# ardaduz/deep-video-mvs

Hardware: AMD Instinct MI355X
Metric: depth frames/sec/GPU @ 320x256x64 planes (fusionnet); rel-L1 vs ref (higher is better)
Workload: dtype f32

## Files before the change

deep-video-mvs_amd/csrc/direct_conv.hip:

```cpp
#include <stdlib.h>

#include "dvmvs_device.h"

namespace dvmvs {

typedef float float4v __attribute__((ext_vector_type(4)));

struct DirectConvArgs {
  const float* x;
  const float* packed;
  const float* bias;
  float* dst;
  float* dst_nhwc;
  long long x_batch_stride, dst_batch_stride;
  int B, C_in, C_out, H, W, OH, OW;
  int act;
  int n_groups;
  int packed_groups;
  int n_chunks;
  int tiles_x;
  int vec4;
};

#ifdef DVMVS_SWEEP_TRACE
// ... 320 lines not shown
}

template <int PX>
__global__ __launch_bounds__(256) void conv_head_kernel(const float* __restrict__ x, const float* __restrict__ w, const float* __restrict__ bias,
                                                        float* __restrict__ dst, long long x_batch_stride, long long dst_batch_stride, int C, int H,
                                                        int W, int act, float p0, float p1) {
  constexpr int SL = 256 / PX;
  __shared__ float s_part[SL][PX];
  const int px = threadIdx.x % PX, slice = threadIdx.x / PX;
  const int HW = H * W;
  const int p = blockIdx.x * PX + px, b = blockIdx.y;
  const int y = p / W, xx = p - y * W;
  const int per = (C + SL - 1) / SL;
  const int c_lo = slice * per, c_hi = min(C, c_lo + per);
  float sum = 0.0f;
  if (p < HW) {
    int off[9];
    bool in[9];
#pragma unroll
    for (int t = 0; t < 9; ++t) {
      const int yy = y + t / 3 - 1, xs = xx + t % 3 - 1;
      in[t] = yy >= 0 && yy < H && xs >= 0 && xs < W;
      off[t] = in[t] ? yy * W + xs : 0;
    }
    const float* xb = x + static_cast<size_t>(b) * x_batch_stride;
#pragma unroll 2
    for (int c = c_lo; c < c_hi; ++c) {
      const float* plane = xb + static_cast<size_t>(c) * HW;
      float v[9];
#pragma unroll
      for (int t = 0; t < 9; ++t) v[t] = in[t] ? plane[off[t]] : 0.0f;
#pragma unroll
      for (int t = 0; t < 9; ++t) sum = fmaf(v[t], w[c * 9 + t], sum);
    }
  }
  s_part[slice][px] = sum;
  __syncthreads();
  if (slice == 0 && p < HW) {
    float total = s_part[0][px];
#pragma unroll
    for (int s = 1; s < SL; ++s) total += s_part[s][px];
    if (bias) total += bias[0];
    dst[static_cast<size_t>(b) * dst_batch_stride + p] = head_activation(total, act, p0, p1);
  }
}

struct DirectConvShape {
  int MW, MT, NT, PW, KS;
};
constexpr DirectConvShape kDcShapes[4] = {{16, 5, 2, 4, 2}, {8, 5, 2, 1, 8}, {16, 5, 1, 1, 8}, {8, 5, 1, 1, 8}};
constexpr int kDcCUs = 256;

inline int direct_conv_choose(int B, int C_in, int C_out, int H, int W, int K, int S) {
  if (B <= 0 || C_in <= 0 || C_out <= 0 || C_out % 16 != 0 || (K != 3 && K != 5) || (S != 1 && S != 2) || H <= 0 || W <= 0) return 0;
  if (S == 2 && (H % 2 != 0 || W % 2 != 0)) return 0;
  const int OH = H / S, OW = W / S;
// ... 110 lines not shown
  a.n_chunks = 0; a.tiles_x = 0;
  hipStream_t s = static_cast<hipStream_t>(stream);
  if (kernel_size == 3) return stride == 1 ? launch_direct_conv_shape<3, 1>(id, a, s) : launch_direct_conv_shape<3, 2>(id, a, s);
  return stride == 1 ? launch_direct_conv_shape<5, 1>(id, a, s) : launch_direct_conv_shape<5, 2>(id, a, s);
}

extern "C" int dvmvs_conv_head_fwd(const float* x, long long x_batch_stride, const float* weight, const float* bias, float* dst,
                                   long long dst_batch_stride, int B, int C_in, int H, int W, int activation, float p0, float p1, dvmvs_stream_t stream) {
  using namespace dvmvs;
  if (!x || !weight || !dst || B <= 0 || C_in <= 0 || H <= 0 || W <= 0) return DVMVS_EINVAL;
  if (activation < 0 || activation > 3) return DVMVS_EINVAL;
  const long long HW = static_cast<long long>(H) * W;
  if (x_batch_stride == 0) x_batch_stride = HW * C_in;
  if (dst_batch_stride == 0) dst_batch_stride = HW;
  hipStream_t s = static_cast<hipStream_t>(stream);
  if (HW >= 16384) {
    hipLaunchKernelGGL((conv_head_kernel<64>), dim3(static_cast<unsigned int>((HW + 63) / 64), B), dim3(256), 0, s, x, weight, bias, dst, x_batch_stride,
                       dst_batch_stride, C_in, H, W, activation, p0, p1);
  } else {
    hipLaunchKernelGGL((conv_head_kernel<16>), dim3(static_cast<unsigned int>((HW + 15) / 16), B), dim3(256), 0, s, x, weight, bias, dst, x_batch_stride,
                       dst_batch_stride, C_in, H, W, activation, p0, p1);
  }
  return launch_status();
}

#ifdef DVMVS_SWEEP_TRACE
extern "C" int dvmvs_debug_direct_conv_trace(unsigned long long* host, int waves) {
  if (waves > dvmvs::kDcTraceWaves) waves = dvmvs::kDcTraceWaves;
  return static_cast<int>(hipMemcpyFromSymbol(host, HIP_SYMBOL(dvmvs::g_dc_trace), sizeof(unsigned long long) * dvmvs::kDcTraceWords * waves));
}
#endif
// ... 1 lines not shown
```

deep-video-mvs_amd/csrc/dvmvs_device.h:

```cpp
#pragma once

#include <hip/hip_runtime.h>
#include <stdint.h>

#include "../../include/dvmvs_hip.h"

namespace dvmvs {

constexpr int kWave = 64;

#define DVMVS_GLOBAL __attribute__((address_space(1)))
typedef const float DVMVS_GLOBAL* gcfloat_p;
typedef float DVMVS_GLOBAL* gfloat_p;
typedef unsigned int DVMVS_GLOBAL* guint_p;
__device__ inline gcfloat_p as_global(const float* p) { return (gcfloat_p)p; }
__device__ inline gfloat_p as_global(float* p) { return (gfloat_p)p; }
__device__ inline guint_p as_global(unsigned int* p) { return (guint_p)p; }

#define DVMVS_RETURN_IF_HIP(expr)                      \
  do {                                                 \
    hipError_t _e = (expr);                            \
    if (_e != hipSuccess) return static_cast<int>(_e); \
  } while (0)

// ... 90 lines not shown
  const float ey = (fy + 1.0f) - ay;
  const float wy = ay - fy;
  t.w_nw = ex * ey;
  t.w_ne = wx * ey;
  t.w_sw = ex * wy;
  t.w_se = wx * wy;
  t.in_x0 = (t.x0 >= 0) && (t.x0 < W);
  t.in_x1 = (t.x0 + 1 >= 0) && (t.x0 + 1 < W);
  t.in_y0 = (t.y0 >= 0) && (t.y0 < H);
  t.in_y1 = (t.y0 + 1 >= 0) && (t.y0 + 1 < H);
  return t;
}

__device__ inline float unnormalize_ac(float g, int size) { return ((g + 1.0f) * 0.5f) * static_cast<float>(size - 1); }

__device__ inline int wave_inclusive_scan(int x) {
  const int lane = threadIdx.x & 63;
#pragma unroll
  for (int off = 1; off < 64; off <<= 1) {
    const int y = __shfl_up(x, off, 64);
    if (lane >= off) x += y;
  }
  return x;
}

template <int kBlock = 256>
__device__ inline int block_exclusive_scan(int v, int* lds, int& total) {
  const int incl = wave_inclusive_scan(v);
  const int wave = threadIdx.x >> 6;
  if ((threadIdx.x & 63) == 63) lds[wave] = incl;
// ... 41 lines not shown
```

deep-video-mvs_amd/csrc/frame_ops.hip:

```cpp
#include "dvmvs_device.h"

namespace dvmvs {

template <int ACT>
__device__ inline float apply_act(float v, float p0 = 0.0f, float p1 = 0.0f) {
  if (ACT == 1) return fmaxf(v, 0.0f);
  if (ACT == 2) return 1.0f / (1.0f + expf(-v));
  if (ACT == 3) {
#pragma clang fp contract(off)
    const float s = 1.0f / (1.0f + expf(-v));
    return 1.0f / (p0 * s + p1);
  }
  return v;
}

template <int ACT, bool VEC4, int RES>
__global__ __launch_bounds__(256) void bias_act_kernel(const float* x, float* dst, long long dst_batch_stride, const float* __restrict__ bias,
                                                       const float* __restrict__ residual, int C, int HW, int W, float p0, float p1) {
  const int plane = blockIdx.y;
  const int b = plane / C, c = plane - b * C;
  const float bv = bias ? bias[c] : 0.0f;
  const float* p = x + static_cast<size_t>(plane) * HW;
  float* d = dst + static_cast<size_t>(b) * dst_batch_stride + static_cast<size_t>(c) * HW;
  if (VEC4 && RES != 2) {
// ... 44 lines not shown
    const long long pl = i / (static_cast<long long>(OW) * OH);
    const float fy = sh * static_cast<float>(oy), fx = sw * static_cast<float>(ox);
    const int y0 = static_cast<int>(fy), x0 = static_cast<int>(fx);
    const int y1 = y0 + (y0 < H - 1 ? 1 : 0), x1 = x0 + (x0 < W - 1 ? 1 : 0);
    const float h1 = fy - static_cast<float>(y0), h0 = 1.0f - h1;
    const float w1 = fx - static_cast<float>(x0), w0 = 1.0f - w1;
    const float* p = in + pl * H * W;
    const long long b = pl / C, c = pl - b * C;
    const float bv = (PRE != 0 && pre_bias) ? pre_bias[c] : 0.0f;
    const float v00 = PRE ? apply_act<PRE>(p[y0 * W + x0] + bv) : p[y0 * W + x0], v01 = PRE ? apply_act<PRE>(p[y0 * W + x1] + bv) : p[y0 * W + x1];
    const float v10 = PRE ? apply_act<PRE>(p[y1 * W + x0] + bv) : p[y1 * W + x0], v11 = PRE ? apply_act<PRE>(p[y1 * W + x1] + bv) : p[y1 * W + x1];
    out[b * out_batch_stride + (c * OH + oy) * OW + ox] = h0 * (w0 * v00 + w1 * v01) + h1 * (w0 * v10 + w1 * v11);
  }
}

template <int PRE>
__device__ inline void upsample2x_quads_plane(const float* __restrict__ in, float* __restrict__ out, long long out_batch_stride, const float* __restrict__ pre_bias,
                                              int pl, int C, int H, int W) {
#pragma clang fp contract(off)
  typedef float float4v __attribute__((ext_vector_type(4)));
  const int OH = 2 * H, OW = 2 * W, QW = OW >> 2;
  const float sh = OH > 1 ? static_cast<float>(H - 1) / static_cast<float>(OH - 1) : 0.0f;
  const float sw = OW > 1 ? static_cast<float>(W - 1) / static_cast<float>(OW - 1) : 0.0f;
  const int b = pl / C, c = pl - b * C;
  const float* p = in + static_cast<size_t>(pl) * H * W;
  const float bv = (PRE != 0 && pre_bias) ? pre_bias[c] : 0.0f;
  float* dst = out + static_cast<size_t>(b) * out_batch_stride + static_cast<size_t>(c) * OH * OW;
  for (int q = blockIdx.x * 256 + threadIdx.x; q < OH * QW; q += gridDim.x * 256) {
    const int oy = q / QW, ox = 4 * (q - oy * QW);
    const float fy = sh * static_cast<float>(oy);
    const int y0 = static_cast<int>(fy);
    const int y1 = y0 + (y0 < H - 1 ? 1 : 0);
    const float h1 = fy - static_cast<float>(y0), h0 = 1.0f - h1;
    const float* r0 = p + y0 * W;
    const float* r1 = p + y1 * W;
    float4v v;
#pragma unroll
    for (int e = 0; e < 4; ++e) {
      const float fx = sw * static_cast<float>(ox + e);
      const int x0 = static_cast<int>(fx);
      const int x1 = x0 + (x0 < W - 1 ? 1 : 0);
      const float w1 = fx - static_cast<float>(x0), w0 = 1.0f - w1;
      const float v00 = PRE ? apply_act<PRE>(r0[x0] + bv) : r0[x0], v01 = PRE ? apply_act<PRE>(r0[x1] + bv) : r0[x1];
      const float v10 = PRE ? apply_act<PRE>(r1[x0] + bv) : r1[x0], v11 = PRE ? apply_act<PRE>(r1[x1] + bv) : r1[x1];
      v[e] = h0 * (w0 * v00 + w1 * v01) + h1 * (w0 * v10 + w1 * v11);
    }
    *reinterpret_cast<float4v*>(dst + oy * OW + ox) = v;
  }
}

template <int PRE>
__global__ __launch_bounds__(256) void upsample2x_quads_kernel(const float* __restrict__ in, float* __restrict__ out, long long out_batch_stride,
                                                               const float* __restrict__ pre_bias, int C, int H, int W) {
  upsample2x_quads_plane<PRE>(in, out, out_batch_stride, pre_bias, blockIdx.y, C, H, W);
}

template <int PRE2>
__global__ __launch_bounds__(256) void upsample2x_pair_quads_kernel(const float* __restrict__ in1, float* __restrict__ out1, long long out1_batch_stride, int C1,
                                                                    const float* __restrict__ in2, float* __restrict__ out2, long long out2_batch_stride,
                                                                    const float* __restrict__ pre_bias2, int C2, int planes1, int H, int W) {
  const int pl = blockIdx.y;
  if (pl < planes1) upsample2x_quads_plane<0>(in1, out1, out1_batch_stride, nullptr, pl, C1, H, W);
  else upsample2x_quads_plane<PRE2>(in2, out2, out2_batch_stride, pre_bias2, pl - planes1, C2, H, W);
}

template <int K, int ACT, bool PRE>
__global__ __launch_bounds__(256) void depthwise_conv_kernel(const float* __restrict__ in, const float* __restrict__ weight,
                                                             const float* __restrict__ bias, const float* __restrict__ pre_bias,
                                                             float* __restrict__ out, int C, int H, int W, int OH, int OW, int stride) {
  const int c = blockIdx.y, b = blockIdx.z;
  const float* wk = weight + static_cast<size_t>(c) * K * K;
  const float* src = in + (static_cast<size_t>(b) * C + c) * H * W;
  float* dst = out + (static_cast<size_t>(b) * C + c) * OH * OW;
  const float bv = bias ? bias[c] : 0.0f;
  const float pv = (PRE && pre_bias) ? pre_bias[c] : 0.0f;
  for (int i = blockIdx.x * blockDim.x + threadIdx.x; i < OH * OW; i += gridDim.x * blockDim.x) {
    const int oy = i / OW, ox = i - oy * OW;
    const int y0 = oy * stride - K / 2, x0 = ox * stride - K / 2;
// ... 144 lines not shown
                     planes <= 65535 && static_cast<long long>(H) * W < (1LL << 27);
  if (!quads) {
    const int rc = dvmvs_upsample2x_fwd(in1, out1, out1_batch_stride, nullptr, 0, B, C1, H, W, stream);
    return rc != 0 ? rc : dvmvs_upsample2x_fwd(in2, out2, out2_batch_stride, pre_bias2, pre_activation2, B, C2, H, W, stream);
  }
  const int n_quads = 2 * H * (W / 2);
  const int per_plane = max(1, min((n_quads + 255) / 256, max(1, 4096 / static_cast<int>(planes))));
  const dim3 grid(static_cast<unsigned>(per_plane), static_cast<unsigned>(planes)), block(256);
  hipStream_t s = static_cast<hipStream_t>(stream);
#define DVMVS_UP2(P) hipLaunchKernelGGL(upsample2x_pair_quads_kernel<P>, grid, block, 0, s, in1, out1, out1_batch_stride, C1, in2, out2, out2_batch_stride, pre_bias2, C2, B * C1, H, W)
  if (pre_activation2 == 1) DVMVS_UP2(1); else if (pre_activation2 == 2) DVMVS_UP2(2); else DVMVS_UP2(0);
#undef DVMVS_UP2
  return launch_status();
}

extern "C" int dvmvs_depthwise_conv_fwd(const float* in, const float* weight, const float* bias, const float* pre_bias, int pre_relu,
                                        float* out, int B, int C, int H, int W, int kernel_size, int stride, int activation,
                                        dvmvs_stream_t stream) {
  using namespace dvmvs;
  if (!in || !weight || !out || B <= 0 || C <= 0 || H <= 0 || W <= 0) return DVMVS_EINVAL;
  if ((kernel_size != 3 && kernel_size != 5) || (stride != 1 && stride != 2) || activation < 0 || activation > 2) return DVMVS_EUNSUPPORTED;
  if (C > 65535 || B > 65535) return DVMVS_EUNSUPPORTED;
  const int pad = kernel_size / 2;
  const int OH = (H + 2 * pad - kernel_size) / stride + 1, OW = (W + 2 * pad - kernel_size) / stride + 1;
  hipStream_t s = static_cast<hipStream_t>(stream);
#define DVMVS_DW(K, A) return launch_depthwise<K, A>(in, weight, bias, pre_bias, pre_relu != 0, out, B, C, H, W, OH, OW, stride, s)
  if (kernel_size == 3) {
    if (activation == 0) DVMVS_DW(3, 0);
    if (activation == 1) DVMVS_DW(3, 1);
    DVMVS_DW(3, 2);
// ... 35 lines not shown
```

deep-video-mvs_amd/dvmvs/engine.py:

```python
import contextlib
import copy
import time
import os
from collections import OrderedDict
from typing import NamedTuple

import torch
from torch import nn

from dvmvs.config import Config
from dvmvs.hip import ops as _ops
from dvmvs import pose_algebra as _pose_algebra
from dvmvs import utils as _utils

import dvmvs as _package
_DETERMINISTIC_MIOPEN = _package.DETERMINISTIC_MIOPEN
_MIOPEN_SWITCH_WAS_PRESET = _package.MIOPEN_SWITCH_WAS_PRESET or os.environ.get("DVMVS_KEEP_MIOPEN_ATOMIC_KERNELS", "0") == "1"

_MAX_MEAS = 8
_STAGING_SLOTS = int(os.environ.get("DVMVS_STAGING_SLOTS", "1"))
_GRAPH_QUEUE_FILLERS = int(os.environ.get("DVMVS_GRAPH_QUEUE_FILLERS", "1"))
def _fork_point(value):
    try:
        level = int(value)
    except (TypeError, ValueError):
        level = None
    if level not in (-1, 0, 1, 2, 3, 4):
        raise ValueError(f"DVMVS_FORK_AFTER must be an integer from -1 to 4, got {value!r}")
    return level


_FORK_AFTER = _fork_point(os.environ.get("DVMVS_FORK_AFTER", "1"))
_PAIRED_UPSAMPLING = os.environ.get("DVMVS_PAIRED_UPSAMPLING", "1") != "0"
_UP2X_IN_CONV = os.environ.get("DVMVS_UP2X_IN_CONV", "1") != "0"
_UPLOAD_IN_COPY_BATCH = os.environ.get("DVMVS_UPLOAD_IN_COPY_BATCH", "1") != "0"
_AUX_STREAM = os.environ.get("DVMVS_AUX_STREAM", "0")
_BATCH_COPIES = os.environ.get("DVMVS_BATCH_COPIES", "1") != "0"


def _fold_pair(conv, bn):
    w = conv.weight
    scale = bn.weight / torch.sqrt(bn.running_var + bn.eps)
    folded = nn.Conv2d(conv.in_channels, conv.out_channels, conv.kernel_size, stride=conv.stride, padding=conv.padding,
                       dilation=conv.dilation, groups=conv.groups, bias=True).to(w.device)
    with torch.no_grad():
        folded.weight.copy_(w * scale.reshape(-1, 1, 1, 1))
        bias = conv.bias if conv.bias is not None else torch.zeros_like(bn.running_mean)
        folded.bias.copy_((bias - bn.running_mean) * scale + bn.bias)
# ... 861 lines not shown
            top = fpn.inner_blocks[level](taps[level], residual=top, residual_mode=2)
            if level == 0 and half_nhwc is not None and isinstance(fpn.layer_blocks[0], FusedConv2d):
                fpn.layer_blocks[0](top, out=outs[0], out_nhwc=half_nhwc)
                half_nhwc = None
            else:
                fpn.layer_blocks[level](top, out=outs[level])
        if half_nhwc is not None:
            _ops.nchw_to_nhwc_into(outs[0], half_nhwc)

    def _decoder_block_direct(self, block, x, cat, depth_head, depth_input):
        up_channels = block.up_convolution.conv[0].weight.shape[0]
        up_conv = block.up_convolution.conv[0]
        if depth_head is not None and _PAIRED_UPSAMPLING and self._aux_stream is None:
            B, C, H, W = x.shape
            up = torch.empty((B, C, 2 * H, 2 * W), device=x.device, dtype=torch.float32)
            _ops.upsample2x_pair_into(x, up, depth_head[0](depth_input, raw=True), cat[:, -1:], depth_head[0].bias, _ops.ACTIVATIONS["sigmoid"])
            up_conv(up, out=cat[:, :up_channels])
            return block.convolution2[0](block.convolution1[0](cat))
        if depth_head is not None:
            with self._beside("heads"):
                self._upsampled_depth_head(depth_head, depth_input, cat[:, -1:])
        if isinstance(up_conv, FusedConv2d):
            up_conv.forward_upsampled(x, out=cat[:, :up_channels])
        else:
            up_conv(_ops.upsample2x(x), out=cat[:, :up_channels])
        self._join_beside()
        return block.convolution2[0](block.convolution1[0](cat))

    @contextlib.contextmanager
    def _beside(self, use):
        aux = self._aux_stream if _AUX_STREAM in ("1", use) else None
        if aux is None:
            yield
            return
        aux.wait_stream(torch.cuda.current_stream(self.device))
        with torch.cuda.stream(aux):
            yield
        self._beside_open = True

    def _join_beside(self):
        if self._aux_stream is not None and getattr(self, "_beside_open", False):
            torch.cuda.current_stream(self.device).wait_stream(self._aux_stream)
            self._beside_open = False

    @staticmethod
    def _upsampled_depth_head(head, x, dst):
        _ops.upsample2x_into(head[0](x, raw=True), dst, head[0].bias, _ops.ACTIVATIONS["sigmoid"])

    def _lstm_bottleneck(self, x):
        if not self.bottleneck_convs:
            return False
        if self._lstm_packed is None:
            conv = self.lstm.lstm_cell.conv
            k = conv.weight.shape
            ok = conv.bias is None and tuple(k[2:]) == (3, 3) and tuple(conv.padding) == (1, 1) and tuple(conv.stride) == (1, 1) and conv.groups == 1
            splits = _ops.bottleneck_conv_splits(x.shape[0], k[0], k[1], x.shape[2], x.shape[3], 1) if ok else 0
            if splits == 0 or torch.cuda.is_current_stream_capturing():
                return False
# ... 122 lines not shown
                    _ops.partial_sums_bias_act_into(self._lstm_partials, splits, self._lstm_combined, None, _ops.ACTIVATIONS["none"],
                                                    tuple(self._lstm_combined.shape))
                    _ops.lstm_gates_into(self._lstm_combined, s["c"], s["h"])
            else:
                combined = cell.conv(lstm_cat)
                if not combined.is_contiguous():
                    combined = combined.contiguous()
                _ops.lstm_gates_into(combined, s["c"], s["h"])
            bottom = s["h"]
        d1 = self._decoder_block_direct(dec.decoder_block1, bottom, dec_cat[0], None, None)
        d2 = self._decoder_block_direct(dec.decoder_block2, d1, dec_cat[1], dec.depth_layer_one_sixteen, d1)
        d3 = self._decoder_block_direct(dec.decoder_block3, d2, dec_cat[2], dec.depth_layer_one_eight, d2)
        d4 = self._decoder_block_direct(dec.decoder_block4, d3, dec_cat[3], dec.depth_layer_quarter, d3)
        full_in = buffers["full_in"]
        if _PAIRED_UPSAMPLING and self._aux_stream is None:
            _ops.upsample2x_pair_into(d4, full_in[:, :32], dec.depth_layer_half[0](d4, raw=True), full_in[:, 32:33], dec.depth_layer_half[0].bias,
                                      _ops.ACTIVATIONS["sigmoid"])
        else:
            with self._beside("heads"):
                self._upsampled_depth_head(dec.depth_layer_half, d4, full_in[:, 32:33])
            _ops.upsample2x_into(d4, full_in[:, :32])
            self._join_beside()
        refined = dec.refine[1][0](dec.refine[0][0](full_in))
        dec.depth_layer_full[0](refined, out=s["prev_depth"], activation=_ops.ACTIVATION_SIGMOID_TO_DEPTH,
                                p0=dec.inverse_depth_multiplier, p1=dec.inverse_depth_base)

    def _frame_body(self, n_meas, has_previous, sweep_variant=0, parity=0, have=0, give=0, n_meas_next=0, next_variant=0):
        if self.direct:
            return self._frame_body_direct(n_meas, has_previous, sweep_variant, parity, have, give, n_meas_next, next_variant)
        s = self._static
        feats = self._features(s["image"])
        ref_half = feats[0].contiguous()
# ... 275 lines not shown
```

deep-video-mvs_amd/dvmvs/hip/_capi.py:

```python
import ctypes
import os
import threading

import torch

_HERE = os.path.dirname(os.path.abspath(__file__))
LIB_PATH = os.environ.get("DVMVS_HIP_LIB", os.path.normpath(os.path.join(_HERE, "..", "..", "lib", "libdvmvs_hip.so")))

ABI_VERSION = 11
MAX_MEASUREMENTS = 8
MAX_DEPTH_LEVELS = 256
LAYOUT_NCHW, LAYOUT_NHWC = 0, 1

_c_fp = ctypes.c_void_p
_c_fpp = ctypes.POINTER(ctypes.c_void_p)
_c_int = ctypes.c_int
_c_dbl = ctypes.c_double
_c_stream = ctypes.c_void_p
_c_f3 = ctypes.POINTER(ctypes.c_float)

SIGNATURES = {
    "dvmvs_abi_version": (_c_int, []),
    "dvmvs_build_arch": (ctypes.c_char_p, []),
    "dvmvs_error_string": (ctypes.c_char_p, [_c_int]),
# ... 38 lines not shown
    "dvmvs_direct_conv_dual_fwd": (_c_int, [_c_fp, ctypes.c_longlong, _c_fp, _c_int, _c_fp, _c_fp, ctypes.c_longlong, _c_fp] + [_c_int] * 8 + [_c_stream]),
    "dvmvs_pointwise_conv_supported": (_c_int, [_c_int] * 7),
    "dvmvs_pointwise_conv_packed_bytes": (ctypes.c_size_t, [_c_int] * 2),
    "dvmvs_pointwise_conv_pack": (_c_int, [_c_fp, _c_fp, _c_int, _c_int, _c_stream]),
    "dvmvs_pointwise_conv_fwd": (_c_int, [_c_fp, ctypes.c_longlong, _c_fp, _c_fp, _c_fp, ctypes.c_longlong, _c_int, _c_fp, ctypes.c_longlong] + [_c_int] * 7 + [_c_stream]),
    "dvmvs_conv_head_fwd": (_c_int, [_c_fp, ctypes.c_longlong, _c_fp, _c_fp, _c_fp, ctypes.c_longlong] + [_c_int] * 5 + [ctypes.c_float, ctypes.c_float, _c_stream]),
    "dvmvs_partial_sums_bias_act_fwd": (_c_int, [_c_fp, _c_int, _c_fp, ctypes.c_longlong, _c_fp, _c_int, _c_int, _c_int, _c_int, _c_stream]),
    "dvmvs_depth_reproject_fwd": (_c_int, [_c_fp, _c_fp, _c_fp, _c_fp, _c_fp, _c_fp, _c_int,
                                           _c_int, _c_int, _c_int, _c_stream]),
    "dvmvs_bias_act_fwd": (_c_int, [_c_fp, _c_fp, ctypes.c_longlong, _c_fp, _c_fp, _c_int, _c_int, _c_int, _c_int, _c_int, _c_int,
                                    ctypes.c_float, ctypes.c_float, _c_stream]),
    "dvmvs_bias_act_inplace": (_c_int, [_c_fp, _c_fp, _c_fp, _c_int, _c_int, _c_int, _c_int, _c_int, _c_int, _c_stream]),
    "dvmvs_conv_bias_act_fwd": (_c_int, [_c_fp, _c_fp, _c_fp, _c_fp, ctypes.c_longlong] + [_c_int] * 9 + [_c_stream]),
    "dvmvs_upsample2x_fwd": (_c_int, [_c_fp, _c_fp, ctypes.c_longlong, _c_fp, _c_int, _c_int, _c_int, _c_int, _c_int, _c_stream]),
    "dvmvs_upsample2x_pair_fwd": (_c_int, [_c_fp, _c_fp, ctypes.c_longlong, _c_int, _c_fp, _c_fp, ctypes.c_longlong, _c_fp, _c_int, _c_int, _c_int, _c_int, _c_int, _c_stream]),
    "dvmvs_upsample2x_bwd": (_c_int, [_c_fp, _c_fp, _c_int, _c_int, _c_int, _c_int, _c_stream]),
    "dvmvs_depthwise_conv_bwd_workspace_bytes": (ctypes.c_size_t, [_c_int] * 6),
    "dvmvs_depthwise_conv_bwd": (_c_int, [_c_fp, _c_fp, _c_fp, _c_fp, _c_fp, _c_fp, _c_int, _c_int, _c_int, _c_int, _c_int, _c_int, _c_stream]),
    "dvmvs_depth_reproject_lowres_fwd": (_c_int, [_c_fp, _c_fp, _c_fp, _c_fp, _c_fp, _c_fp, _c_int, _c_int, _c_int, _c_int, _c_stream]),
    "dvmvs_depth_reproject_estimate_fwd": (_c_int, [_c_fp, _c_fp, _c_fp, _c_fp, _c_fp, _c_fp, _c_int, _c_int, _c_int, _c_int, _c_stream]),
    "dvmvs_tsdf_integrate": (_c_int, [_c_fp, _c_fp, _c_fp, _c_int, _c_int, _c_int, ctypes.c_float, ctypes.c_float, ctypes.c_float,
                                      ctypes.c_float, _c_fp, _c_fp, _c_fp, _c_fp, _c_int, _c_int, ctypes.c_float, ctypes.c_float, _c_stream]),
    "dvmvs_marching_cubes_workspace_bytes": (ctypes.c_size_t, [_c_int, _c_int, _c_int]),
    "dvmvs_marching_cubes_count": (_c_int, [_c_fp, _c_int, _c_int, _c_int, ctypes.c_float, _c_fp, ctypes.c_size_t, _c_fp, _c_stream]),
    "dvmvs_marching_cubes_emit": (_c_int, [_c_fp, _c_fp, _c_int, _c_int, _c_int, ctypes.c_float, ctypes.c_float, ctypes.c_float,
                                           ctypes.c_float, ctypes.c_float, _c_fp, _c_fp, _c_fp, _c_fp, _c_fp, ctypes.c_longlong,
                                           ctypes.c_longlong, _c_stream]),
    "dvmvs_depthwise_conv_fwd": (_c_int, [_c_fp, _c_fp, _c_fp, _c_fp, _c_int, _c_fp, _c_int, _c_int, _c_int, _c_int, _c_int, _c_int, _c_int,
                                          _c_stream]),
    "dvmvs_rgb_sweep_fwd": (_c_int, [_c_fp, _c_fpp, _c_fp, _c_fp, _c_fp, _c_int, _c_int, _c_int, _c_int, _c_int, _c_int,
# ... 32 lines not shown
    "dvmvs_voxel_keys": (_c_int, [_c_fp, ctypes.c_longlong, ctypes.c_float, _c_fp, ctypes.c_size_t, _c_fp, _c_stream]),
    "dvmvs_voxel_downsample_count": (_c_int, [_c_fp, ctypes.c_longlong, _c_fp, _c_fp, _c_fp, ctypes.c_size_t, _c_fp, _c_stream]),
    "dvmvs_voxel_downsample_emit": (_c_int, [ctypes.c_longlong, ctypes.c_longlong, _c_fp, _c_fp, _c_fp, _c_stream]),
}

ADDED_WITHIN_ABI = ("dvmvs_preprocess_rgb_fwd", "dvmvs_preprocess_depth_fwd")
ADDED_WITHIN_ABI_DEPTH_ERRORS = ("dvmvs_depth_errors_workspace_bytes", "dvmvs_depth_errors_fwd")
ADDED_WITHIN_ABI_TSDF_RAYCAST = ("dvmvs_tsdf_raycast_mask_bytes", "dvmvs_tsdf_raycast_mask", "dvmvs_tsdf_raycast_fwd")
ADDED_WITHIN_ABI_TSDF_FUSE = ("dvmvs_tsdf_integrate_frames_workspace_bytes", "dvmvs_tsdf_integrate_frames")
ADDED_WITHIN_ABI_NEAREST = ("dvmvs_nearest_workspace_bytes", "dvmvs_nearest_query_workspace_bytes", "dvmvs_nearest_build",
                            "dvmvs_nearest_distance_fwd", "dvmvs_distance_metrics_fwd")
ADDED_WITHIN_ABI_CONSISTENCY = ("dvmvs_consistency_matrices", "dvmvs_depth_consistency_fwd")
ADDED_WITHIN_ABI_SURFACE_SAMPLE = ("dvmvs_surface_sample_workspace_bytes", "dvmvs_surface_sample_count", "dvmvs_surface_sample_emit",
                                   "dvmvs_voxel_downsample_workspace_bytes", "dvmvs_voxel_keys", "dvmvs_voxel_downsample_count",
                                   "dvmvs_voxel_downsample_emit")

_lib = None
_lock = threading.Lock()


def lib():
    global _lib
    if _lib is not None:
        return _lib
    with _lock:
        if _lib is not None:
            return _lib
        if not os.path.exists(LIB_PATH):
            raise RuntimeError(
                f"dvmvs HIP library not found at {LIB_PATH}. Build it with `make -C deep-video-mvs_amd/csrc` "
                f"(or __graft_entry__.build()). The plane-sweep ops have no CPU / eager fallback.")
        handle = ctypes.CDLL(LIB_PATH)
        added = (ADDED_WITHIN_ABI + ADDED_WITHIN_ABI_DEPTH_ERRORS + ADDED_WITHIN_ABI_TSDF_RAYCAST + ADDED_WITHIN_ABI_TSDF_FUSE
                 + ADDED_WITHIN_ABI_NEAREST + ADDED_WITHIN_ABI_CONSISTENCY + ADDED_WITHIN_ABI_SURFACE_SAMPLE)
        missing = [name for name in added if not hasattr(handle, name)]
        if missing:
            raise RuntimeError(f"{LIB_PATH} was built before {', '.join(missing)} joined ABI {ABI_VERSION} (the number did not change); "
                               f"rebuild it with `make -C deep-video-mvs_amd/csrc` (or __graft_entry__.build())")
        for name, (restype, argtypes) in SIGNATURES.items():
            fn = getattr(handle, name)
            fn.restype = restype
            fn.argtypes = argtypes
        got = handle.dvmvs_abi_version()
        if got != ABI_VERSION:
            raise RuntimeError(f"libdvmvs_hip.so ABI {got} does not match the Python binding ({ABI_VERSION}); rebuild")
        _lib = handle
    return _lib


# ... 16 lines not shown
```

deep-video-mvs_amd/dvmvs/hip/ops/frame.py:

```python
import ctypes
from typing import Optional, Tuple

import torch
from torch import Tensor

from dvmvs.hip import _capi
from dvmvs.hip.ops._common import EUNSUPPORTED, channel_ptr, check_tensors, custom_op, launch, opt_ptr, ptr

ACTIVATIONS = {"none": 0, "relu": 1, "sigmoid": 2}
ACTIVATION_SIGMOID_TO_DEPTH = 3
RESIDUAL_NONE, RESIDUAL_SAME, RESIDUAL_NEAREST_UP2 = 0, 1, 2


@custom_op("hidden_warp", fake=lambda image_src, depth_dst, src_trans_dst, camera_matrix, zero_invalid: torch.empty_like(image_src))
def hidden_warp(image_src: Tensor, depth_dst: Tensor, src_trans_dst: Tensor, camera_matrix: Tensor,
                zero_invalid: bool) -> Tensor:
    check_tensors("hidden_warp", image_src, depth_dst, src_trans_dst, camera_matrix)
    B, C, H, W = image_src.shape
    image_src = image_src.contiguous()
    out = torch.empty_like(image_src)
    launch("dvmvs_hidden_warp_fwd", image_src.device, ptr(image_src), ptr(depth_dst.contiguous()), ptr(src_trans_dst.contiguous()),
           ptr(camera_matrix.contiguous()), ptr(out), B, C, H, W, int(bool(zero_invalid)))
    return out

# ... 329 lines not shown


def upsample2x_pair_into(x1: Tensor, dst1: Tensor, x2: Tensor, dst2: Tensor, pre_bias2=None, pre_activation2: int = 0) -> None:
    check_tensors("upsample2x_pair_into", x1, x2)
    x1, x2 = x1.contiguous(), x2.contiguous()
    B, C1, H, W = x1.shape
    C2 = x2.shape[1]
    if tuple(x2.shape) != (B, C2, H, W):
        raise ValueError(f"dvmvs::upsample2x_pair_into: the two maps must have the same batch and size, got {tuple(x1.shape)} and {tuple(x2.shape)}")
    stride1 = _slice_batch_stride("upsample2x_pair_into", dst1, B, C1, 2 * H, 2 * W)
    stride2 = _slice_batch_stride("upsample2x_pair_into", dst2, B, C2, 2 * H, 2 * W)
    launch("dvmvs_upsample2x_pair_fwd", x1.device, ptr(x1), ptr(dst1), stride1, C1, ptr(x2), ptr(dst2), stride2,
           channel_ptr("upsample2x_pair_into", "pre_bias2", pre_bias2, C2), int(pre_activation2), C2, B, H, W)


def bottleneck_conv_splits(B: int, C_out: int, C_in: int, H_in: int, W_in: int, stride: int) -> int:
    n = _capi.lib().dvmvs_bottleneck_conv_splits(int(B), int(C_out), int(C_in), int(H_in), int(W_in), int(stride))
    return n if n > 0 else 0


def _packed_weights(entry, weight, nbytes, *args):
    packed = torch.empty(nbytes // 4, dtype=torch.float32, device=weight.device)
    launch(entry, weight.device, ptr(weight.contiguous()), ptr(packed), *args)
    return packed


def bottleneck_conv_pack(weight: Tensor) -> Tensor:
    check_tensors("bottleneck_conv_pack", weight)
    C_out, C_in, kh, kw = weight.shape
    nbytes = _capi.lib().dvmvs_bottleneck_conv_packed_bytes(C_out, C_in) if (kh, kw) == (3, 3) else 0
# ... 118 lines not shown
```

include/dvmvs_hip.h:

```cpp
#ifndef DVMVS_HIP_H
#define DVMVS_HIP_H

#include <stddef.h>
#include <stdint.h>

#ifdef __cplusplus
extern "C" {
#endif

#define DVMVS_ABI_VERSION 11
#define DVMVS_MAX_MEASUREMENTS 8
#define DVMVS_MAX_DEPTH_LEVELS 256

#define DVMVS_LAYOUT_NCHW 0
#define DVMVS_LAYOUT_NHWC 1

#define DVMVS_EINVAL (-1)
#define DVMVS_EUNSUPPORTED (-2)
#define DVMVS_ELIBRARY (-3)

typedef void* dvmvs_stream_t;

int dvmvs_abi_version(void);
const char* dvmvs_build_arch(void);
// ... 98 lines not shown
                                     int B, int full_height, int full_width, dvmvs_stream_t stream);

int dvmvs_depth_reproject_estimate_fwd(const float* transformation, const float* previous_depth, const float* full_K,
                                       const float* half_K, float* estimate, float* estimate_to_clear, int lowres_factor,
                                       int B, int full_height, int full_width, dvmvs_stream_t stream);

int dvmvs_bias_act_fwd(const float* x, float* dst, long long dst_batch_stride, const float* bias, const float* residual,
                       int residual_mode, int B, int C, int H, int W, int activation, float p0, float p1, dvmvs_stream_t stream);
int dvmvs_bias_act_inplace(float* x, const float* bias, const float* residual, int residual_mode, int B, int C, int H, int W,
                           int activation, dvmvs_stream_t stream);
int dvmvs_upsample2x_fwd(const float* in, float* out, long long out_batch_stride, const float* pre_bias, int pre_activation,
                         int B, int C, int H, int W, dvmvs_stream_t stream);
int dvmvs_upsample2x_pair_fwd(const float* in1, float* out1, long long out1_batch_stride, int C1, const float* in2, float* out2,
                              long long out2_batch_stride, const float* pre_bias2, int pre_activation2, int C2, int B, int H, int W,
                              dvmvs_stream_t stream);
int dvmvs_conv_bias_act_fwd(const float* x, const float* weight, const float* bias, float* out, long long out_batch_stride,
                            int B, int Cin, int H, int W, int Cout, int K, int stride, int padding, int activation, dvmvs_stream_t stream);
int dvmvs_depthwise_conv_fwd(const float* in, const float* weight, const float* bias, const float* pre_bias, int pre_relu, float* out,
                             int B, int C, int H, int W, int kernel_size, int stride, int activation, dvmvs_stream_t stream);

int dvmvs_tsdf_integrate(float* tsdf_vol, float* weight_vol, float* color_vol, int dim_x, int dim_y, int dim_z,
                         float origin_x, float origin_y, float origin_z, float voxel_size, const float* cam_intr,
                         const float* cam_pose, const float* color_im, const float* depth_im, int im_h, int im_w,
                         float trunc_margin, float obs_weight, dvmvs_stream_t stream);

size_t dvmvs_marching_cubes_workspace_bytes(int X, int Y, int Z);
int dvmvs_marching_cubes_count(const float* vol, int X, int Y, int Z, float level, void* workspace, size_t workspace_bytes,
                               long long* counts_dev, dvmvs_stream_t stream);
int dvmvs_marching_cubes_emit(const float* vol, const float* color_vol, int X, int Y, int Z, float level, float ox, float oy, float oz,
                              float voxel_size, void* workspace, float* verts, float* normals, unsigned char* colors, int* faces,
// ... 69 lines not shown
```

Before: 1419.

## Fuse depth-head 3x3 conv into paired upsample kernel via tiled LDS recompute

Adds a fused kernel that computes the single-channel 3x3 depth-head convolution per output tile into shared memory, then bilinearly upsamples it with bias and sigmoid, alongside the plain feature-map upsample in the same launch. This removes a separate head conv launch and its intermediate low-res write and read at each decoder scale. Shared helpers are factored out of the existing head conv and upsample code. Tiles recompute halo pixels, which costs some redundant conv work and extra syncs per tile, and the engine falls back to the old path when shapes are unsupported.

Result: faster. 1438 (median of 6 runs) (+1.3%).

```diff
diff --git a/deep-video-mvs_amd/csrc/direct_conv.hip b/deep-video-mvs_amd/csrc/direct_conv.hip
--- a/deep-video-mvs_amd/csrc/direct_conv.hip
+++ b/deep-video-mvs_amd/csrc/direct_conv.hip
@@ -358,32 +358,11 @@
   const int per = (C + SL - 1) / SL;
   const int c_lo = slice * per, c_hi = min(C, c_lo + per);
   float sum = 0.0f;
-  if (p < HW) {
-    int off[9];
-    bool in[9];
-#pragma unroll
-    for (int t = 0; t < 9; ++t) {
-      const int yy = y + t / 3 - 1, xs = xx + t % 3 - 1;
-      in[t] = yy >= 0 && yy < H && xs >= 0 && xs < W;
-      off[t] = in[t] ? yy * W + xs : 0;
-    }
-    const float* xb = x + static_cast<size_t>(b) * x_batch_stride;
-#pragma unroll 2
-    for (int c = c_lo; c < c_hi; ++c) {
-      const float* plane = xb + static_cast<size_t>(c) * HW;
-      float v[9];
-#pragma unroll
-      for (int t = 0; t < 9; ++t) v[t] = in[t] ? plane[off[t]] : 0.0f;
-#pragma unroll
-      for (int t = 0; t < 9; ++t) sum = fmaf(v[t], w[c * 9 + t], sum);
-    }
-  }
+  if (p < HW) sum = conv_head_slice<2>(x + static_cast<size_t>(b) * x_batch_stride, w, c_lo, c_hi, y, xx, H, W);
   s_part[slice][px] = sum;
   __syncthreads();
   if (slice == 0 && p < HW) {
-    float total = s_part[0][px];
-#pragma unroll
-    for (int s = 1; s < SL; ++s) total += s_part[s][px];
+    float total = conv_head_add_slices<SL>(&s_part[0][px], PX);
     if (bias) total += bias[0];
     dst[static_cast<size_t>(b) * dst_batch_stride + p] = head_activation(total, act, p0, p1);
   }
@@ -524,7 +503,7 @@
   if (x_batch_stride == 0) x_batch_stride = HW * C_in;
   if (dst_batch_stride == 0) dst_batch_stride = HW;
   hipStream_t s = static_cast<hipStream_t>(stream);
-  if (HW >= 16384) {
+  if (conv_head_pixels(HW) == 64) {
     hipLaunchKernelGGL((conv_head_kernel<64>), dim3(static_cast<unsigned int>((HW + 63) / 64), B), dim3(256), 0, s, x, weight, bias, dst, x_batch_stride,
                        dst_batch_stride, C_in, H, W, activation, p0, p1);
   } else {
diff --git a/deep-video-mvs_amd/csrc/dvmvs_device.h b/deep-video-mvs_amd/csrc/dvmvs_device.h
--- a/deep-video-mvs_amd/csrc/dvmvs_device.h
+++ b/deep-video-mvs_amd/csrc/dvmvs_device.h
@@ -128,6 +128,40 @@
 
 __device__ inline float unnormalize_ac(float g, int size) { return ((g + 1.0f) * 0.5f) * static_cast<float>(size - 1); }
 
+inline int conv_head_pixels(long long HW) { return HW >= 16384 ? 64 : 16; }
+
+template <int UNROLL>
+__device__ inline float conv_head_slice(const float* __restrict__ xb, const float* __restrict__ w, int c_lo, int c_hi, int y, int xx, int H, int W) {
+  const int HW = H * W;
+  int off[9];
+  bool in[9];
+#pragma unroll
+  for (int t = 0; t < 9; ++t) {
+    const int yy = y + t / 3 - 1, xs = xx + t % 3 - 1;
+    in[t] = yy >= 0 && yy < H && xs >= 0 && xs < W;
+    off[t] = in[t] ? yy * W + xs : 0;
+  }
+  float sum = 0.0f;
+#pragma unroll UNROLL
+  for (int c = c_lo; c < c_hi; ++c) {
+    const float* plane = xb + static_cast<size_t>(c) * HW;
+    float v[9];
+#pragma unroll
+    for (int t = 0; t < 9; ++t) v[t] = in[t] ? plane[off[t]] : 0.0f;
+#pragma unroll
+    for (int t = 0; t < 9; ++t) sum = fmaf(v[t], w[c * 9 + t], sum);
+  }
+  return sum;
+}
+
+template <int SL>
+__device__ inline float conv_head_add_slices(const float* part, int stride) {
+  float total = part[0];
+#pragma unroll
+  for (int s = 1; s < SL; ++s) total += part[s * stride];
+  return total;
+}
+
 __device__ inline int wave_inclusive_scan(int x) {
   const int lane = threadIdx.x & 63;
 #pragma unroll
diff --git a/deep-video-mvs_amd/csrc/frame_ops.hip b/deep-video-mvs_amd/csrc/frame_ops.hip
--- a/deep-video-mvs_amd/csrc/frame_ops.hip
+++ b/deep-video-mvs_amd/csrc/frame_ops.hip
@@ -82,38 +82,53 @@
   }
 }
 
+typedef float float4v __attribute__((ext_vector_type(4)));
+
+__device__ inline float upsample2x_scale(int n) {
+  return 2 * n > 1 ? static_cast<float>(n - 1) / static_cast<float>(2 * n - 1) : 0.0f;
+}
+
+__device__ inline void upsample2x_taps(float scale, int o, int n, int& i0, int& i1, float& l1) {
+#pragma clang fp contract(off)
+  const float f = scale * static_cast<float>(o);
+  i0 = static_cast<int>(f);
+  i1 = i0 + (i0 < n - 1 ? 1 : 0);
+  l1 = f - static_cast<float>(i0);
+}
+
+template <int PRE>
+__device__ inline float4v upsample2x_quad(const float* __restrict__ r0, const float* __restrict__ r1, float h1, float sw, float bv, int ox, int W) {
+#pragma clang fp contract(off)
+  const float h0 = 1.0f - h1;
+  float4v v;
+#pragma unroll
+  for (int e = 0; e < 4; ++e) {
+    int x0, x1;
+    float w1;
+    upsample2x_taps(sw, ox + e, W, x0, x1, w1);
+    const float w0 = 1.0f - w1;
+    const float v00 = PRE ? apply_act<PRE>(r0[x0] + bv) : r0[x0], v01 = PRE ? apply_act<PRE>(r0[x1] + bv) : r0[x1];
+    const float v10 = PRE ? apply_act<PRE>(r1[x0] + bv) : r1[x0], v11 = PRE ? apply_act<PRE>(r1[x1] + bv) : r1[x1];
+    v[e] = h0 * (w0 * v00 + w1 * v01) + h1 * (w0 * v10 + w1 * v11);
+  }
+  return v;
+}
+
 template <int PRE>
 __device__ inline void upsample2x_quads_plane(const float* __restrict__ in, float* __restrict__ out, long long out_batch_stride, const float* __restrict__ pre_bias,
                                               int pl, int C, int H, int W) {
-#pragma clang fp contract(off)
-  typedef float float4v __attribute__((ext_vector_type(4)));
   const int OH = 2 * H, OW = 2 * W, QW = OW >> 2;
-  const float sh = OH > 1 ? static_cast<float>(H - 1) / static_cast<float>(OH - 1) : 0.0f;
-  const float sw = OW > 1 ? static_cast<float>(W - 1) / static_cast<float>(OW - 1) : 0.0f;
+  const float sh = upsample2x_scale(H), sw = upsample2x_scale(W);
   const int b = pl / C, c = pl - b * C;
   const float* p = in + static_cast<size_t>(pl) * H * W;
   const float bv = (PRE != 0 && pre_bias) ? pre_bias[c] : 0.0f;
   float* dst = out + static_cast<size_t>(b) * out_batch_stride + static_cast<size_t>(c) * OH * OW;
   for (int q = blockIdx.x * 256 + threadIdx.x; q < OH * QW; q += gridDim.x * 256) {
     const int oy = q / QW, ox = 4 * (q - oy * QW);
-    const float fy = sh * static_cast<float>(oy);
-    const int y0 = static_cast<int>(fy);
-    const int y1 = y0 + (y0 < H - 1 ? 1 : 0);
-    const float h1 = fy - static_cast<float>(y0), h0 = 1.0f - h1;
-    const float* r0 = p + y0 * W;
-    const float* r1 = p + y1 * W;
-    float4v v;
-#pragma unroll
-    for (int e = 0; e < 4; ++e) {
-      const float fx = sw * static_cast<float>(ox + e);
-      const int x0 = static_cast<int>(fx);
-      const int x1 = x0 + (x0 < W - 1 ? 1 : 0);
-      const float w1 = fx - static_cast<float>(x0), w0 = 1.0f - w1;
-      const float v00 = PRE ? apply_act<PRE>(r0[x0] + bv) : r0[x0], v01 = PRE ? apply_act<PRE>(r0[x1] + bv) : r0[x1];
-      const float v10 = PRE ? apply_act<PRE>(r1[x0] + bv) : r1[x0], v11 = PRE ? apply_act<PRE>(r1[x1] + bv) : r1[x1];
-      v[e] = h0 * (w0 * v00 + w1 * v01) + h1 * (w0 * v10 + w1 * v11);
-    }
-    *reinterpret_cast<float4v*>(dst + oy * OW + ox) = v;
+    int y0, y1;
+    float h1;
+    upsample2x_taps(sh, oy, H, y0, y1, h1);
+    *reinterpret_cast<float4v*>(dst + oy * OW + ox) = upsample2x_quad<PRE>(p + y0 * W, p + y1 * W, h1, sw, bv, ox, W);
   }
 }
 
@@ -130,6 +145,76 @@
   const int pl = blockIdx.y;
   if (pl < planes1) upsample2x_quads_plane<0>(in1, out1, out1_batch_stride, nullptr, pl, C1, H, W);
   else upsample2x_quads_plane<PRE2>(in2, out2, out2_batch_stride, pre_bias2, pl - planes1, C2, H, W);
+}
+
+template <int PX>
+struct HeadTile {
+  static constexpr int TR = PX == 16 ? 6 : 14, TC = PX == 16 ? 4 : 12;
+  static constexpr int MAX_R = TR / 2 + 3, MAX_C = TC / 2 + 2, WIN = MAX_R * MAX_C;
+};
+
+inline int head_tiles(int n, int tile, int lead) { return (n + lead + tile - 1) / tile; }
+
+template <int PX, int PRE2>
+__device__ inline void upsample2x_head_tile(const float* __restrict__ x2, long long x2_batch_stride, const float* __restrict__ w2, const float* __restrict__ bias2,
+                                            float* __restrict__ out2, long long out2_batch_stride, int C2, int H, int W, int tile, int tiles_r, int tiles_c) {
+  typedef HeadTile<PX> T;
+  constexpr int SL = 256 / PX;
+  __shared__ float lds[256 + T::WIN];
+  float* s_part = lds;
+  float* s_val = lds + 256;
+  const int OH = 2 * H, OW = 2 * W;
+  const int b = tile / (tiles_r * tiles_c), tr = (tile / tiles_c) % tiles_r, tc = tile % tiles_c;
+  const int oy_lo = max(0, tr * T::TR - 1), oy_hi = min(OH, (tr + 1) * T::TR - 1);
+  const int ox_lo = tc * T::TC, ox_hi = min(OW, (tc + 1) * T::TC);
+  const float sh = upsample2x_scale(H), sw = upsample2x_scale(W);
+  int y_lo, y_hi, x_lo, x_hi, unused;
+  float l1;
+  upsample2x_taps(sh, oy_lo, H, y_lo, unused, l1);
+  upsample2x_taps(sh, oy_hi - 1, H, unused, y_hi, l1);
+  upsample2x_taps(sw, ox_lo, W, x_lo, unused, l1);
+  upsample2x_taps(sw, ox_hi - 1, W, unused, x_hi, l1);
+  const int n_cols = x_hi - x_lo + 1, n = (y_hi - y_lo + 1) * n_cols;
+  if (y_hi - y_lo + 1 > T::MAX_R || n_cols > T::MAX_C) return;
+
+  const int px = threadIdx.x % PX, slice = threadIdx.x / PX;
+  const int per = (C2 + SL - 1) / SL;
+  const int c_lo = slice * per, c_hi = min(C2, c_lo + per);
+  const float* xb = x2 + static_cast<size_t>(b) * x2_batch_stride;
+  for (int first = 0; first < n; first += PX) {
+    const int i = first + px;
+    float sum = 0.0f;
+    if (i < n) sum = conv_head_slice<4>(xb, w2, c_lo, c_hi, y_lo + i / n_cols, x_lo + i % n_cols, H, W);
+    s_part[slice * PX + px] = sum;
+    __syncthreads();
+    if (slice == 0 && i < n) s_val[i] = conv_head_add_slices<SL>(s_part + px, PX);
+    __syncthreads();
+  }
+
+  const float bv = (PRE2 != 0 && bias2) ? bias2[0] : 0.0f;
+  float* dst = out2 + static_cast<size_t>(b) * out2_batch_stride;
+  const int qw = (ox_hi - ox_lo) >> 2;
+  for (int q = threadIdx.x; q < (oy_hi - oy_lo) * qw; q += 256) {
+    const int oy = oy_lo + q / qw, ox = ox_lo + 4 * (q % qw);
+    int y0, y1;
+    float h1;
+    upsample2x_taps(sh, oy, H, y0, y1, h1);
+    *reinterpret_cast<float4v*>(dst + oy * OW + ox) =
+        upsample2x_quad<PRE2>(s_val + (y0 - y_lo) * n_cols - x_lo, s_val + (y1 - y_lo) * n_cols - x_lo, h1, sw, bv, ox, W);
+  }
+}
+
+template <int PX, int PRE2>
+__global__ __launch_bounds__(256) void upsample2x_pair_head_kernel(const float* __restrict__ in1, float* __restrict__ out1, long long out1_batch_stride, int C1,
+                                                                   const float* __restrict__ x2, long long x2_batch_stride, const float* __restrict__ w2,
+                                                                   const float* __restrict__ bias2, float* __restrict__ out2, long long out2_batch_stride,
+                                                                   int C2, int H, int W, int tiles_y, int n_tiles, int tiles_r, int tiles_c) {
+  if (static_cast<int>(blockIdx.y) >= tiles_y) {
+    upsample2x_quads_plane<0>(in1, out1, out1_batch_stride, nullptr, blockIdx.y - tiles_y, C1, H, W);
+    return;
+  }
+  const int tile = blockIdx.y * gridDim.x + blockIdx.x;
+  if (tile < n_tiles) upsample2x_head_tile<PX, PRE2>(x2, x2_batch_stride, w2, bias2, out2, out2_batch_stride, C2, H, W, tile, tiles_r, tiles_c);
 }
 
 template <int K, int ACT, bool PRE>
@@ -304,6 +389,46 @@
   return launch_status();
 }
 
+template <int PX>
+static int launch_pair_head(const float* in1, float* out1, long long out1_batch_stride, int C1, const float* x2, long long x2_batch_stride, const float* weight2,
+                            const float* bias2, int pre_activation2, int C2, float* out2, long long out2_batch_stride, int B, int H, int W, hipStream_t s) {
+  using namespace dvmvs;
+  const long long planes1 = static_cast<long long>(B) * C1;
+  const int n_quads = 2 * H * (W / 2);
+  const int per_plane = max(1, min((n_quads + 255) / 256, max(1, 4096 / static_cast<int>(planes1 + B))));
+  const int tiles_r = head_tiles(2 * H, HeadTile<PX>::TR, 1), tiles_c = head_tiles(2 * W, HeadTile<PX>::TC, 0);
+  const long long n_tiles = static_cast<long long>(B) * tiles_r * tiles_c;
+  const long long tiles_y = (n_tiles + per_plane - 1) / per_plane;
+  if (tiles_y + planes1 > 65535) return DVMVS_EUNSUPPORTED;
+  const dim3 grid(static_cast<unsigned>(per_plane), static_cast<unsigned>(tiles_y + planes1)), block(256);
+#define DVMVS_UP2H(P)                                                                                                                                \
+  hipLaunchKernelGGL((upsample2x_pair_head_kernel<PX, P>), grid, block, 0, s, in1, out1, out1_batch_stride, C1, x2, x2_batch_stride, weight2, bias2, out2, \
+                     out2_batch_stride, C2, H, W, static_cast<int>(tiles_y), static_cast<int>(n_tiles), tiles_r, tiles_c)
+  if (pre_activation2 == 1) DVMVS_UP2H(1); else if (pre_activation2 == 2) DVMVS_UP2H(2); else DVMVS_UP2H(0);
+#undef DVMVS_UP2H
+  return launch_status();
+}
+
+extern "C" int dvmvs_upsample2x_pair_head_fwd(const float* in1, float* out1, long long out1_batch_stride, int C1, const float* x2, long long x2_batch_stride,
+                                              const float* weight2, const float* bias2, int pre_activation2, int C2, float* out2,
+                                              long long out2_batch_stride, int B, int H, int W, dvmvs_stream_t stream) {
+  using namespace dvmvs;
+  if (!in1 || !out1 || !x2 || !weight2 || !out2 || B <= 0 || C1 <= 0 || C2 <= 0 || H <= 0 || W <= 0) return DVMVS_EINVAL;
+  if (pre_activation2 < 0 || pre_activation2 > 2) return DVMVS_EINVAL;
+  const long long HW = static_cast<long long>(H) * W;
+  if (out1_batch_stride == 0) out1_batch_stride = HW * 4 * C1;
+  if (out2_batch_stride == 0) out2_batch_stride = HW * 4;
+  if (x2_batch_stride == 0) x2_batch_stride = HW * C2;
+  if (out1_batch_stride < HW * 4 * C1 || out2_batch_stride < HW * 4 || x2_batch_stride < HW * C2) return DVMVS_EINVAL;
+  if (W % 2 != 0 || ((reinterpret_cast<uintptr_t>(out1) | reinterpret_cast<uintptr_t>(out2)) & 15) != 0 || ((out1_batch_stride | out2_batch_stride) & 3) != 0 ||
+      HW >= (1LL << 27) || H >= (1 << 22) || W >= (1 << 22) || static_cast<long long>(B) * (C1 + 1) > 65535)
+    return DVMVS_EUNSUPPORTED;
+  hipStream_t s = static_cast<hipStream_t>(stream);
+  if (conv_head_pixels(HW) == 64)
+    return launch_pair_head<64>(in1, out1, out1_batch_stride, C1, x2, x2_batch_stride, weight2, bias2, pre_activation2, C2, out2, out2_batch_stride, B, H, W, s);
+  return launch_pair_head<16>(in1, out1, out1_batch_stride, C1, x2, x2_batch_stride, weight2, bias2, pre_activation2, C2, out2, out2_batch_stride, B, H, W, s);
+}
+
 extern "C" int dvmvs_depthwise_conv_fwd(const float* in, const float* weight, const float* bias, const float* pre_bias, int pre_relu,
                                         float* out, int B, int C, int H, int W, int kernel_size, int stride, int activation,
                                         dvmvs_stream_t stream) {
diff --git a/deep-video-mvs_amd/dvmvs/engine.py b/deep-video-mvs_amd/dvmvs/engine.py
--- a/deep-video-mvs_amd/dvmvs/engine.py
+++ b/deep-video-mvs_amd/dvmvs/engine.py
@@ -32,6 +32,14 @@
 
 _FORK_AFTER = _fork_point(os.environ.get("DVMVS_FORK_AFTER", "1"))
 _PAIRED_UPSAMPLING = os.environ.get("DVMVS_PAIRED_UPSAMPLING", "1") != "0"
+def _switch(name, default):
+    value = os.environ.get(name, default)
+    if value not in ("0", "1"):
+        raise ValueError(f"{name} must be 0 or 1, got {value!r}")
+    return value == "1"
+
+
+_HEAD_IN_UPSAMPLER = _switch("DVMVS_HEAD_IN_UPSAMPLER", "1")
 _UP2X_IN_CONV = os.environ.get("DVMVS_UP2X_IN_CONV", "1") != "0"
 _UPLOAD_IN_COPY_BATCH = os.environ.get("DVMVS_UPLOAD_IN_COPY_BATCH", "1") != "0"
 _AUX_STREAM = os.environ.get("DVMVS_AUX_STREAM", "0")
@@ -923,7 +931,7 @@
         if depth_head is not None and _PAIRED_UPSAMPLING and self._aux_stream is None:
             B, C, H, W = x.shape
             up = torch.empty((B, C, 2 * H, 2 * W), device=x.device, dtype=torch.float32)
-            _ops.upsample2x_pair_into(x, up, depth_head[0](depth_input, raw=True), cat[:, -1:], depth_head[0].bias, _ops.ACTIVATIONS["sigmoid"])
+            self._upsample_pair_with_head(x, up, depth_head[0], depth_input, cat[:, -1:])
             up_conv(up, out=cat[:, :up_channels])
             return block.convolution2[0](block.convolution1[0](cat))
         if depth_head is not None:
@@ -951,6 +959,17 @@
         if self._aux_stream is not None and getattr(self, "_beside_open", False):
             torch.cuda.current_stream(self.device).wait_stream(self._aux_stream)
             self._beside_open = False
+
+    @staticmethod
+    def _upsample_pair_with_head(x, dst, head, head_input, head_dst):
+        sigmoid = _ops.ACTIVATIONS["sigmoid"]
+        k = head.weight.shape
+        if _HEAD_IN_UPSAMPLER and isinstance(head, FusedConv2d) and head.direct_conv and tuple(k) == (1, head_input.shape[1], 3, 3) and head.groups == 1 \
+                and tuple(head.stride) == (1, 1) and tuple(head.padding) == (1, 1) and tuple(head.dilation) == (1, 1) \
+                and x.is_contiguous() and head_input.is_contiguous() and head_input.data_ptr() % 16 == 0:
+            if _ops.frame._upsample2x_pair_head_into(x, dst, head_input, head.weight, head_dst, head.bias, sigmoid):
+                return
+        _ops.upsample2x_pair_into(x, dst, head(head_input, raw=True), head_dst, head.bias, sigmoid)
 
     @staticmethod
     def _upsampled_depth_head(head, x, dst):
@@ -1103,8 +1122,7 @@
         d4 = self._decoder_block_direct(dec.decoder_block4, d3, dec_cat[3], dec.depth_layer_quarter, d3)
         full_in = buffers["full_in"]
         if _PAIRED_UPSAMPLING and self._aux_stream is None:
-            _ops.upsample2x_pair_into(d4, full_in[:, :32], dec.depth_layer_half[0](d4, raw=True), full_in[:, 32:33], dec.depth_layer_half[0].bias,
-                                      _ops.ACTIVATIONS["sigmoid"])
+            self._upsample_pair_with_head(d4, full_in[:, :32], dec.depth_layer_half[0], d4, full_in[:, 32:33])
         else:
             with self._beside("heads"):
                 self._upsampled_depth_head(dec.depth_layer_half, d4, full_in[:, 32:33])
diff --git a/deep-video-mvs_amd/dvmvs/hip/_capi.py b/deep-video-mvs_amd/dvmvs/hip/_capi.py
--- a/deep-video-mvs_amd/dvmvs/hip/_capi.py
+++ b/deep-video-mvs_amd/dvmvs/hip/_capi.py
@@ -76,6 +76,8 @@
     "dvmvs_conv_bias_act_fwd": (_c_int, [_c_fp, _c_fp, _c_fp, _c_fp, ctypes.c_longlong] + [_c_int] * 9 + [_c_stream]),
     "dvmvs_upsample2x_fwd": (_c_int, [_c_fp, _c_fp, ctypes.c_longlong, _c_fp, _c_int, _c_int, _c_int, _c_int, _c_int, _c_stream]),
     "dvmvs_upsample2x_pair_fwd": (_c_int, [_c_fp, _c_fp, ctypes.c_longlong, _c_int, _c_fp, _c_fp, ctypes.c_longlong, _c_fp, _c_int, _c_int, _c_int, _c_int, _c_int, _c_stream]),
+    "dvmvs_upsample2x_pair_head_fwd": (_c_int, [_c_fp, _c_fp, ctypes.c_longlong, _c_int, _c_fp, ctypes.c_longlong, _c_fp, _c_fp, _c_int, _c_int, _c_fp, ctypes.c_longlong,
+                                                _c_int, _c_int, _c_int, _c_stream]),
     "dvmvs_upsample2x_bwd": (_c_int, [_c_fp, _c_fp, _c_int, _c_int, _c_int, _c_int, _c_stream]),
     "dvmvs_depthwise_conv_bwd_workspace_bytes": (ctypes.c_size_t, [_c_int] * 6),
     "dvmvs_depthwise_conv_bwd": (_c_int, [_c_fp, _c_fp, _c_fp, _c_fp, _c_fp, _c_fp, _c_int, _c_int, _c_int, _c_int, _c_int, _c_int, _c_stream]),
@@ -138,6 +140,7 @@
 ADDED_WITHIN_ABI_SURFACE_SAMPLE = ("dvmvs_surface_sample_workspace_bytes", "dvmvs_surface_sample_count", "dvmvs_surface_sample_emit",
                                    "dvmvs_voxel_downsample_workspace_bytes", "dvmvs_voxel_keys", "dvmvs_voxel_downsample_count",
                                    "dvmvs_voxel_downsample_emit")
+ADDED_WITHIN_ABI_DECODER = ("dvmvs_upsample2x_pair_head_fwd",)
 
 _lib = None
 _lock = threading.Lock()
@@ -156,7 +159,7 @@
                 f"(or __graft_entry__.build()). The plane-sweep ops have no CPU / eager fallback.")
         handle = ctypes.CDLL(LIB_PATH)
         added = (ADDED_WITHIN_ABI + ADDED_WITHIN_ABI_DEPTH_ERRORS + ADDED_WITHIN_ABI_TSDF_RAYCAST + ADDED_WITHIN_ABI_TSDF_FUSE
-                 + ADDED_WITHIN_ABI_NEAREST + ADDED_WITHIN_ABI_CONSISTENCY + ADDED_WITHIN_ABI_SURFACE_SAMPLE)
+                 + ADDED_WITHIN_ABI_NEAREST + ADDED_WITHIN_ABI_CONSISTENCY + ADDED_WITHIN_ABI_SURFACE_SAMPLE + ADDED_WITHIN_ABI_DECODER)
         missing = [name for name in added if not hasattr(handle, name)]
         if missing:
             raise RuntimeError(f"{LIB_PATH} was built before {', '.join(missing)} joined ABI {ABI_VERSION} (the number did not change); "
diff --git a/deep-video-mvs_amd/dvmvs/hip/ops/frame.py b/deep-video-mvs_amd/dvmvs/hip/ops/frame.py
--- a/deep-video-mvs_amd/dvmvs/hip/ops/frame.py
+++ b/deep-video-mvs_amd/dvmvs/hip/ops/frame.py
@@ -367,6 +367,26 @@
            channel_ptr("upsample2x_pair_into", "pre_bias2", pre_bias2, C2), int(pre_activation2), C2, B, H, W)
 
 
+def _upsample2x_pair_head_into(x1: Tensor, dst1: Tensor, x2: Tensor, weight2: Tensor, dst2: Tensor, bias2=None, pre_activation2: int = 0) -> bool:
+    check_tensors("upsample2x_pair_head_into", x1, x2, weight2)
+    B, C1, H, W = x1.shape
+    C2 = x2.shape[1]
+    if not (x1.is_contiguous() and x2.is_contiguous() and weight2.is_contiguous()) or tuple(x2.shape) != (B, C2, H, W) or \
+            tuple(weight2.shape) != (1, C2, 3, 3):
+        raise ValueError(f"dvmvs::upsample2x_pair_head_into: expected contiguous maps of the same batch and size and a [1,{C2},3,3] weight, got "
+                         f"{tuple(x1.shape)}, {tuple(x2.shape)}, {tuple(weight2.shape)}")
+    stride1 = _slice_batch_stride("upsample2x_pair_head_into", dst1, B, C1, 2 * H, 2 * W)
+    stride2 = _slice_batch_stride("upsample2x_pair_head_into", dst2, B, 1, 2 * H, 2 * W)
+    with torch.cuda.device(x1.device):
+        rc = _capi.lib().dvmvs_upsample2x_pair_head_fwd(ptr(x1), ptr(dst1), stride1, C1, ptr(x2), 0, ptr(weight2),
+                                                        channel_ptr("upsample2x_pair_head_into", "bias2", bias2, 1), int(pre_activation2), C2,
+                                                        ptr(dst2), stride2, B, H, W, torch.cuda.current_stream(x1.device).cuda_stream)
+    if rc == EUNSUPPORTED:
+        return False
+    _capi.check(rc, "dvmvs_upsample2x_pair_head_fwd")
+    return True
+
+
 def bottleneck_conv_splits(B: int, C_out: int, C_in: int, H_in: int, W_in: int, stride: int) -> int:
     n = _capi.lib().dvmvs_bottleneck_conv_splits(int(B), int(C_out), int(C_in), int(H_in), int(W_in), int(stride))
     return n if n > 0 else 0
diff --git a/include/dvmvs_hip.h b/include/dvmvs_hip.h
--- a/include/dvmvs_hip.h
+++ b/include/dvmvs_hip.h
@@ -136,6 +136,9 @@
 int dvmvs_upsample2x_pair_fwd(const float* in1, float* out1, long long out1_batch_stride, int C1, const float* in2, float* out2,
                               long long out2_batch_stride, const float* pre_bias2, int pre_activation2, int C2, int B, int H, int W,
                               dvmvs_stream_t stream);
+int dvmvs_upsample2x_pair_head_fwd(const float* in1, float* out1, long long out1_batch_stride, int C1, const float* x2, long long x2_batch_stride,
+                                   const float* weight2, const float* bias2, int pre_activation2, int C2, float* out2,
+                                   long long out2_batch_stride, int B, int H, int W, dvmvs_stream_t stream);
 int dvmvs_conv_bias_act_fwd(const float* x, const float* weight, const float* bias, float* out, long long out_batch_stride,
                             int B, int Cin, int H, int W, int Cout, int K, int stride, int padding, int activation, dvmvs_stream_t stream);
 int dvmvs_depthwise_conv_fwd(const float* in, const float* weight, const float* bias, const float* pre_bias, int pre_relu, float* out,
```
